# powdr-labs/powdr

Measured on AMD Instinct MI355X. Metric: STARK cells/sec (trace rows x cols) proving guest-keccak [bus interactions (LogUp) inside the proof], higher is better.
Workload: dtype u32 (BabyBear, Montgomery)

## Files before the change

include/powdr_prover.h:

```cpp
#ifndef POWDR_PROVER_H
#define POWDR_PROVER_H

#include <stddef.h>
#include <stdint.h>

#ifdef __cplusplus
extern "C" {
#endif

typedef struct PwProver PwProver;

typedef struct {
    uint32_t num_queries;
    uint32_t pow_bits;
} PwStarkConfig;

PwProver* pw_prover_create(const PwStarkConfig* cfg, uint32_t width, const uint32_t* cons_bytecode,
                           size_t bytecode_len, const uint32_t* cons_spans, size_t n_constraints);
PwProver* pw_prover_create_logup(const PwStarkConfig* cfg, uint32_t width, const uint32_t* cons_bytecode,
                                 size_t bytecode_len, const uint32_t* cons_spans, size_t n_constraints,
                                 const uint32_t* interactions, size_t n_interactions, const uint32_t* inter_spans,
                                 size_t n_inter_spans, const uint32_t* inter_bytecode, size_t inter_bytecode_len);
int pw_prover_trace_root(PwProver* p, const uint32_t* d_trace, uint32_t log_height, uint32_t* root8);
int pw_prover_set_bus_seed(PwProver* p, const uint32_t* seed8);
// ... 221 lines not shown
                               uint32_t* total_chunks);
void pw_jit_cache_stats(uint64_t* units_compiled, uint64_t* units_from_disk);
int pw_jit_compile_check(uint32_t width, const uint32_t* cons_bytecode, size_t bytecode_len, const uint32_t* cons_spans, size_t n_constraints,
                         const uint32_t* interactions, size_t n_interactions, const uint32_t* inter_spans, size_t n_inter_spans,
                         const uint32_t* inter_bytecode, size_t inter_bytecode_len, size_t* n_kernels, size_t* code_bytes, size_t* n_chunks,
                         char* err, size_t err_cap);

uint32_t pw_prover_width(const PwProver* p);

size_t pw_prover_device_bytes(const PwProver* p);


int pw_lde_batch(const uint32_t* d_trace, uint32_t width, uint32_t log_height, uint32_t* d_coeffs, uint32_t* d_lde);

int pw_lde_fused(const uint32_t* d_trace, uint32_t width, uint32_t log_height, uint32_t* d_tmp, uint32_t* d_lde);

int pw_lde_subcoset(const uint32_t* d_coeffs, uint32_t width, uint32_t log_height, uint32_t log_blocks, uint32_t r, uint32_t* d_scale,
                    uint32_t* d_out);

int pw_merkle_commit(const uint32_t* d_matrix, size_t height, uint32_t width, uint32_t* d_digests);

void pw_poseidon2_permute_host(uint32_t* state16);

int pw_set_poseidon2_constants(const uint32_t* ext_rc, const uint32_t* int_rc);
void pw_get_poseidon2_constants(uint32_t* ext_rc, uint32_t* int_rc, uint32_t* diag);

#ifdef __cplusplus
}
#endif
#endif
```

powdr_amd/csrc/field_selftest.hpp:

```cpp
#pragma once
#include "ext.hpp"
#include "poseidon2.hpp"

namespace pw {

PW_HD int field_selftest_checks(uint64_t seed, uint32_t iterations) {
    using namespace bb;
    uint64_t s = seed ? seed : 1;
    auto rnd = [&]() { s += 0x9E3779B97F4A7C15ull; uint64_t z = s; z = (z ^ (z >> 30)) * 0xBF58476D1CE4E5B9ull; z = (z ^ (z >> 27)) * 0x94D049BB133111EBull; return z ^ (z >> 31); };
    auto rp = [&]() { return (uint32_t)(rnd() % P); };
    const uint64_t edges64[] = {0, 1, P - 1, P, P + 1, 2ull * P - 1, 2ull * P, 16ull * P - 1, 75ull * P, 128ull * P - 1};
    for (uint64_t x : edges64) {
        if (x < 16ull * P && reduce_sum(x) != x % P) return 1;
        const uint32_t l = reduce_wide_loose(x);
        if (l % P != x % P || l >= (uint64_t)P + P / 32) return 2;
        if (reduce_wide(x) != x % P) return 3;
    }
    const uint32_t edges[] = {0, 1, P - 1, P, P + 1, 2 * P - 1};
    for (uint32_t a : edges)
        for (uint32_t b : edges) {
            const uint32_t r = add_2p(a, b), d = sub_2p(a, b);
            if (r >= 2 * P || r % P != (uint32_t)(((uint64_t)a + b) % P)) return 4;
            if (d >= 2 * P || d % P != (uint32_t)(((uint64_t)a + 2ull * P - b) % P)) return 5;
        }
// ... 26 lines not shown
        }
        const int32_t kappa = it < 3 ? ((it & 1) ? (int32_t)(P / 2) : -(int32_t)(P / 2)) : centred(rp());
        const int32_t rho = it < 3 ? ((it & 2) ? (int32_t)(P / 2) : -(int32_t)(P / 2)) : centred(rp());
        const uint32_t next = it < 3 ? P - 1 : rp(), ex = it < 3 ? (P + 1) / 2 : rp();
        int64_t exit_c[16];
        for (int i = 0; i < 16; ++i) exit_c[i] = (int64_t)centred(ex) * (int64_t)R_MOD_P;
        const bool last = it & 1;
        uint32_t wide = mul(mul(smodp(st[0]), smodp(kappa)), R2_MOD_P);
        for (int i = 1; i < 16; ++i) wide = add(wide, smodp(st[i]));
        const uint32_t sum = mul(wide, 1u);
        const uint32_t sum_r = mul(mul(sum, smodp(rho)), R2_MOD_P);
        for (int i = 0; i < 16; ++i) {
            const uint32_t prod = mul(mul(smodp(st[i]), smodp(m[i])), R2_MOD_P);
            const uint32_t c = i ? (last ? mul(mul(smodp(centred(ex)), R_MOD_P), R2_MOD_P) : 0u) : mul(mul(smodp(centred(next)), R_MOD_P), R2_MOD_P);
            want[i] = mul(add(add(sum_r, prod), c), 1u);
        }
        if (last) p2::internal_layer<true>(st, m, kappa, rho, (int64_t)centred(next) * (int64_t)R_MOD_P, exit_c);
        else p2::internal_layer<false>(st, m, kappa, rho, (int64_t)centred(next) * (int64_t)R_MOD_P, exit_c);
        for (int i = 0; i < 16; ++i)
            if (smodp(st[i]) != want[i]) return 9;
        for (int i = 0; i < 16; ++i)
            if (st[i] <= -(int32_t)P || st[i] >= (int32_t)P) return 9;
    }
    for (uint32_t it = 0; it < iterations; ++it) {
        const uint32_t a = rp(), b = rp(), c = rp(), d = rp();
        {
            const int32_t x = (int32_t)((int64_t)(rnd() % (2ull * P + P / 11)) - (int64_t)(P + P / 22));
            uint32_t want = R_MOD_P;
            for (int k = 0; k < 7; ++k) want = mul(want, smodp(x));
            if (smodp(p2::sbox7(x)) != want) return 8;
            const int64_t y = (int64_t)(rnd() % (128ull * P)) - 64ll * P;
            if (smodp(sreduce_wide_loose(y)) != smodp(y)) return 8;
        }
        const uint32_t ab = mul(a, b);
        if (ab >= P || (uint64_t)ab * R_MOD_P % P != (uint64_t)a * b % P) return 10;
        const uint32_t m2 = mul2(a, b, c, d);
        if (m2 != add(ab, mul(c, d))) return 11;
        const uint32_t la = (uint32_t)(rnd() % (2ull * P));
        const uint32_t ml = mul_lazy(la, b);
        if (ml >= 2 * P || ml % P != mul(la % P, b)) return 12;
        if (add_2p(la, (uint32_t)(rnd() % (2ull * P))) >= 2 * P) return 13;
        const uint64_t w = rnd() % (128ull * P);
        if (reduce_wide(w) != w % P) return 14;
        const uint32_t loose = reduce_wide_loose(w);
        if (loose % P != w % P || loose >= (uint64_t)P + P / 32) return 15;
        const uint64_t w16 = rnd() % (16ull * P);
// ... 49 lines not shown
```

powdr_amd/csrc/merkle.hip:

```cpp
#include "prover_internal.hpp"

#include <algorithm>
#include <cstdlib>
#include <mutex>

namespace pw {

namespace {

constexpr int kBlock = 256;
__constant__ p2::Params c_params;
p2::Params g_host_params;
bool g_params_ready = false;
uint64_t g_params_uploaded = 0;

template <int MINW>
__global__ __launch_bounds__(kBlock, MINW) void leaf_hash_kernel(const uint32_t* __restrict__ m, size_t height,
                                                            uint32_t width, size_t col_stride,
                                                            uint32_t* __restrict__ digests, size_t dstride, size_t doff) {
    const size_t j = (size_t)blockIdx.x * kBlock + threadIdx.x;
    if (j >= height) return;
    uint32_t st[16];
#pragma unroll
    for (int i = 0; i < 16; ++i) st[i] = 0u;
    const uint32_t* col = m + j;
#pragma unroll 1
    for (uint32_t c0 = 0; c0 < width; c0 += 8) {
#pragma unroll
        for (int k = 0; k < 8; ++k)
            if (c0 + k < width) st[k] = col[(size_t)(c0 + k) * col_stride];
        p2::permute<true>(st, c_params);
    }
#pragma unroll
    for (int k = 0; k < 8; ++k) st[k] = bb::reduce_2p(st[k]);
    uint4* out = reinterpret_cast<uint4*>(digests + (j * dstride + doff) * 8);
    out[0] = make_uint4(st[0], st[1], st[2], st[3]);
    out[1] = make_uint4(st[4], st[5], st[6], st[7]);
}

struct LeafLevel {
    const uint32_t* const* cols;
    uint32_t n_cols;
    uint32_t first_block;
    uint64_t height;
    uint32_t* out;
};
struct LeafLevels {
    LeafLevel lv[28];
    int n;
};
template <int MINW>
__global__ __launch_bounds__(kBlock, MINW) void leaf_hash_levels_kernel(const LeafLevels levels) {
    int k = 0;
    while (k + 1 < levels.n && blockIdx.x >= levels.lv[k + 1].first_block) ++k;
    const LeafLevel lv = levels.lv[k];
    const size_t j = (size_t)(blockIdx.x - lv.first_block) * kBlock + threadIdx.x;
    if (j >= lv.height) return;
    uint32_t st[16];
#pragma unroll
    for (int i = 0; i < 16; ++i) st[i] = 0u;
#pragma unroll 1
    for (uint32_t c0 = 0; c0 < lv.n_cols; c0 += 8) {
#pragma unroll
        for (int q = 0; q < 8; ++q)
            if (c0 + q < lv.n_cols) st[q] = lv.cols[c0 + q][j];
        p2::permute<true>(st, c_params);
    }
#pragma unroll
    for (int q = 0; q < 8; ++q) st[q] = bb::reduce_2p(st[q]);
    uint4* out = reinterpret_cast<uint4*>(lv.out + j * 8);
    out[0] = make_uint4(st[0], st[1], st[2], st[3]);
    out[1] = make_uint4(st[4], st[5], st[6], st[7]);
}

struct AbsorbArgs {
    const uint32_t* m;
    size_t col_stride;
    const uint32_t* const* cols;
    uint32_t n_cols, pos0;
    size_t height;
    size_t rstride, roff;
    uint32_t* state;
    uint32_t* digests;
    int first, last;
};
template <int MINW>
__global__ __launch_bounds__(kBlock, MINW) void leaf_absorb_kernel(const AbsorbArgs a) {
    const size_t j = (size_t)blockIdx.x * kBlock + threadIdx.x;
    if (j >= a.height) return;
    const size_t row = j * a.rstride + a.roff;
    uint32_t st[16];
    if (a.first) {
#pragma unroll
        for (int i = 0; i < 16; ++i) st[i] = 0u;
    } else {
        const uint4* in = reinterpret_cast<const uint4*>(a.state + row * 16);
#pragma unroll
        for (int v = 0; v < 4; ++v) { const uint4 x = in[v]; st[4 * v] = x.x; st[4 * v + 1] = x.y; st[4 * v + 2] = x.z; st[4 * v + 3] = x.w; }
    }
    auto cell = [&](uint32_t c) -> uint32_t { return a.cols ? a.cols[c][j] : a.m[(size_t)c * a.col_stride + j]; };
    uint32_t c = 0, pos = a.pos0;
    if (pos) {
#pragma unroll
        for (int k = 0; k < 8; ++k)
            if ((uint32_t)k >= pos && (uint32_t)k - pos < a.n_cols) st[k] = cell((uint32_t)k - pos);
        const uint32_t take = 8u - pos < a.n_cols ? 8u - pos : a.n_cols;
        c = take;
        pos += take;
        if (pos == 8u) { p2::permute<true>(st, c_params); pos = 0; }
    }
#pragma unroll 1
    for (; c < a.n_cols; c += 8) {
#pragma unroll
        for (int k = 0; k < 8; ++k)
            if (c + k < a.n_cols) st[k] = cell(c + k);
        if (c + 8 <= a.n_cols) p2::permute<true>(st, c_params);
        else pos = a.n_cols - c;
    }
    if (a.last) {
        if (pos) p2::permute<true>(st, c_params);
        uint4* out = reinterpret_cast<uint4*>(a.digests + row * 8);
        out[0] = make_uint4(bb::reduce_2p(st[0]), bb::reduce_2p(st[1]), bb::reduce_2p(st[2]), bb::reduce_2p(st[3]));
        out[1] = make_uint4(bb::reduce_2p(st[4]), bb::reduce_2p(st[5]), bb::reduce_2p(st[6]), bb::reduce_2p(st[7]));
    } else {
        uint4* out = reinterpret_cast<uint4*>(a.state + row * 16);
#pragma unroll
        for (int v = 0; v < 4; ++v) out[v] = make_uint4(st[4 * v], st[4 * v + 1], st[4 * v + 2], st[4 * v + 3]);
    }
}

__global__ __launch_bounds__(kBlock) void compress_strided_kernel(const uint32_t* __restrict__ children, size_t n,
                                                                   const uint32_t* __restrict__ inject, uint32_t* __restrict__ parents) {
    const size_t j = (size_t)blockIdx.x * kBlock + threadIdx.x;
    if (j >= n) return;
    const uint4* l = reinterpret_cast<const uint4*>(children + j * 8);
    const uint4* r = reinterpret_cast<const uint4*>(children + (j + n) * 8);
    uint4 a = l[0], b = l[1], c = r[0], d = r[1];
    uint32_t st[16] = {a.x, a.y, a.z, a.w, b.x, b.y, b.z, b.w, c.x, c.y, c.z, c.w, d.x, d.y, d.z, d.w};
    p2::permute(st, c_params);
    if (inject) {
        const uint4* q = reinterpret_cast<const uint4*>(inject + j * 8);
        c = q[0]; d = q[1];
        st[8] = c.x; st[9] = c.y; st[10] = c.z; st[11] = c.w; st[12] = d.x; st[13] = d.y; st[14] = d.z; st[15] = d.w;
        p2::permute(st, c_params);
    }
    uint4* out = reinterpret_cast<uint4*>(parents + j * 8);
    out[0] = make_uint4(st[0], st[1], st[2], st[3]);
    out[1] = make_uint4(st[4], st[5], st[6], st[7]);
}

__global__ __launch_bounds__(kBlock) void ext_pair_leaf_kernel(const bb::Ext* __restrict__ v, size_t half,
                                                                uint32_t* __restrict__ digests) {
    const size_t i = (size_t)blockIdx.x * kBlock + threadIdx.x;
    if (i >= half) return;
    uint32_t st[16];
    const bb::Ext a = v[i], b = v[i + half];
#pragma unroll
    for (int k = 0; k < 4; ++k) { st[k] = a.c[k]; st[4 + k] = b.c[k]; st[8 + k] = 0u; st[12 + k] = 0u; }
    p2::permute(st, c_params);
    uint4* out = reinterpret_cast<uint4*>(digests + i * 8);
    out[0] = make_uint4(st[0], st[1], st[2], st[3]);
    out[1] = make_uint4(st[4], st[5], st[6], st[7]);
}

__global__ __launch_bounds__(kBlock) void compress_kernel(const uint32_t* __restrict__ children, size_t n_parents,
                                                           uint32_t* __restrict__ parents) {
    const size_t i = (size_t)blockIdx.x * kBlock + threadIdx.x;
    if (i >= n_parents) return;
    const uint4* in = reinterpret_cast<const uint4*>(children + i * 16);
    uint4 a = in[0], b = in[1], c = in[2], d = in[3];
    uint32_t st[16] = {a.x, a.y, a.z, a.w, b.x, b.y, b.z, b.w, c.x, c.y, c.z, c.w, d.x, d.y, d.z, d.w};
    p2::permute(st, c_params);
    uint4* out = reinterpret_cast<uint4*>(parents + i * 8);
    out[0] = make_uint4(st[0], st[1], st[2], st[3]);
    out[1] = make_uint4(st[4], st[5], st[6], st[7]);
}

__global__ __launch_bounds__(kBlock) void pow_kernel(const uint32_t* __restrict__ state16, const uint32_t* __restrict__ pending,
                                                      uint32_t in_len, uint32_t bits, uint32_t base, uint32_t* best) {
    const uint32_t w = base + blockIdx.x * kBlock + threadIdx.x;
    if (w >= bb::P) return;
    uint32_t st[16];
#pragma unroll
    for (int i = 0; i < 16; ++i) st[i] = state16[i];
#pragma unroll
    for (int i = 0; i < 8; ++i)
        if ((uint32_t)i < in_len) st[i] = pending[i];
#pragma unroll
    for (int i = 0; i < 8; ++i)
        if ((uint32_t)i == in_len) st[i] = bb::to_monty(w);
    p2::permute(st, c_params);
    const uint32_t sample = st[7];
    if ((bb::from_monty(sample) & ((1u << bits) - 1u)) == 0u) atomicMin(best, w);
}

constexpr size_t kTailNodes = 2048;
__global__ __launch_bounds__(1024) void compress_tail_kernel(uint32_t* __restrict__ digests, size_t n_first, uint32_t* __restrict__ root_out) {
    size_t off = 0;
    for (size_t n = n_first; n > 1; n >>= 1) {
        const size_t parents = n >> 1;
        for (size_t i = threadIdx.x; i < parents; i += 1024) {
            const uint32_t* in = digests + off + i * 16;
            uint32_t st[16];
#pragma unroll
            for (int k = 0; k < 16; ++k) st[k] = in[k];
            p2::permute(st, c_params);
            uint32_t* out = digests + off + n * 8 + i * 8;
#pragma unroll
            for (int k = 0; k < 8; ++k) out[k] = st[k];
        }
        off += n * 8;
        __threadfence_block();
        __syncthreads();
    }
// ... 192 lines not shown
```

powdr_amd/csrc/poseidon2.hpp:

```cpp
#pragma once
#include "babybear.hpp"

#ifndef PW_P2_UNROLL
#define PW_P2_UNROLL 1
#endif
#define PW_P2_STR2(x) #x
#define PW_P2_STR(x) PW_P2_STR2(x)
#define PW_P2_ROUND_LOOP _Pragma(PW_P2_STR(unroll PW_P2_UNROLL))
#ifndef PW_P2_UNROLL_PARTIAL
#define PW_P2_UNROLL_PARTIAL 1
#endif
#define PW_P2_PARTIAL_LOOP _Pragma(PW_P2_STR(unroll PW_P2_UNROLL_PARTIAL))

namespace p2 {

struct Params {
    uint32_t ext_rc[8][16];
    uint32_t int_rc[13];
    uint32_t diag[16];
    int64_t ext_fold[8][16];
    int32_t entry_c;
    int32_t part_kappa[2];
    int32_t part_rho[2];
    int32_t part_diag[2][16];
// ... 73 lines not shown
        p.part_rho[k] = bb::centred((uint32_t)mulm(ratio, mulm(Rm, Rm)));
        for (int i = 0; i < 16; ++i) p.part_diag[k][i] = bb::centred((uint32_t)mulm(p.diag[i], i ? ratio : ratio0));
    }
    for (int r = 0; r < 13; ++r) {
        const uint32_t c = r < 12 ? p.int_rc[r + 1] : p.ext_rc[4][0];
        p.int_fold[r] = (int64_t)bb::centred((uint32_t)mulm(c, lam_second)) * (int64_t)bb::R_MOD_P;
    }
    for (int i = 0; i < 16; ++i) p.exit_fold[i] = i ? (int64_t)bb::centred((uint32_t)mulm(p.ext_rc[4][i], lam_second)) * (int64_t)bb::R_MOD_P : 0;
}

inline void generate_params(Params& p) {
    default_round_constants(p);
    derive_params(p);
}

PW_HD int32_t sbox7(int32_t x) {
    const int32_t x2 = bb::smont(bb::smul(x, x));
    const int32_t x3 = bb::smont(bb::smul(x2, x));
    const int32_t x4 = bb::smont(bb::smul(x2, x2));
    return bb::smont(bb::smul(x3, x4));
}

template <bool FOLD, bool BIAS>
PW_HD void external_layer(int32_t* s, const int64_t* fold) {
    int64_t y[16];
    constexpr int64_t kBias = 4 * (int64_t)bb::P;
#pragma unroll
    for (int b = 0; b < 4; ++b) {
        const int32_t x0 = s[4 * b], x1 = s[4 * b + 1], x2 = s[4 * b + 2], x3 = s[4 * b + 3];
        const int64_t t01 = bb::swide_add(FOLD ? bb::swide_fma_uniform(fold[4 * b], x0, 1) : BIAS ? bb::swide_fma_uniform(kBias, x0, 1) : bb::swide_mul(x0, 1), x1);
        const int64_t t23 = bb::swide_add(FOLD ? bb::swide_fma_uniform(fold[4 * b + 1], x2, 1) : BIAS ? bb::swide_fma_uniform(kBias, x2, 1) : bb::swide_mul(x2, 1), x3);
        const int64_t t = t01 + t23;
        const int64_t ta = bb::swide_add(t, x1), tb = bb::swide_add(t, x3);
        y[4 * b] = ta + t01;
        y[4 * b + 1] = bb::swide_fma(ta, x2, 2) + (FOLD ? fold[4 * b + 2] : (int64_t)0);
        y[4 * b + 2] = tb + t23;
        y[4 * b + 3] = bb::swide_fma(tb, x0, 2) + (FOLD ? fold[4 * b + 3] : (int64_t)0);
    }
#pragma unroll
    for (int i = 0; i < 4; ++i) {
        const int64_t col = (y[i] + y[4 + i]) + (y[8 + i] + y[12 + i]);
#pragma unroll
        for (int b = 0; b < 4; ++b) s[4 * b + i] = BIAS ? bb::sreduce_wide_loose(y[4 * b + i] + col) : bb::smont(y[4 * b + i] + col);
    }
}

template <bool LAST>
PW_HD void internal_layer(int32_t* s, const int32_t* m, int32_t kappa, int32_t rho, int64_t next_c, const int64_t* exit_c) {
    int64_t wide = bb::smul_uniform(s[0], kappa);
#pragma unroll
    for (int i = 1; i < 16; ++i) wide = bb::swide_add(wide, s[i]);
    const int32_t sum = bb::smont(wide);
    const int64_t sum_r = bb::smul_uniform(sum, rho);
    s[0] = bb::smont(bb::swide_mad_uniform(sum_r + next_c, s[0], m[0]));
#pragma unroll
    for (int i = 1; i < 16; ++i) s[i] = bb::smont(bb::swide_mad_uniform(LAST ? sum_r + exit_c[i] : sum_r, s[i], m[i]));
}

template <bool SPONGE = false>
PW_HD void permute(uint32_t* words, const Params& P) {
    int32_t* s = reinterpret_cast<int32_t*>(words);
    external_layer<true, false>(s, P.ext_fold[0]);
PW_P2_ROUND_LOOP
    for (int r = 0; r < 3; ++r) {
#pragma unroll
        for (int i = 0; i < 16; ++i) s[i] = sbox7(s[i]);
        external_layer<true, false>(s, P.ext_fold[r + 1]);
    }
#pragma unroll
    for (int i = 0; i < 16; ++i) s[i] = sbox7(s[i]);
    external_layer<false, false>(s, nullptr);
    s[0] += P.entry_c;
    s[0] = sbox7(s[0]);
    internal_layer<false>(s, P.part_diag[0], P.part_kappa[0], P.part_rho[0], P.int_fold[0], nullptr);
PW_P2_PARTIAL_LOOP
    for (int r = 1; r < 12; ++r) {
        s[0] = sbox7(s[0]);
        internal_layer<false>(s, P.part_diag[1], P.part_kappa[1], P.part_rho[1], P.int_fold[r], nullptr);
    }
    s[0] = sbox7(s[0]);
    internal_layer<true>(s, P.part_diag[1], P.part_kappa[1], P.part_rho[1], P.int_fold[12], P.exit_fold);
PW_P2_ROUND_LOOP
    for (int r = 4; r < 7; ++r) {
#pragma unroll
        for (int i = 0; i < 16; ++i) s[i] = sbox7(s[i]);
        external_layer<true, false>(s, P.ext_fold[r + 1]);
    }
#pragma unroll
    for (int i = 0; i < 16; ++i) s[i] = sbox7(s[i]);
    external_layer<false, true>(s, nullptr);
    if (!SPONGE) {
#pragma unroll
        for (int i = 0; i < 16; ++i) words[i] = bb::reduce_2p(words[i]);
    }
}

}
```

powdr_amd/csrc/prover.hip:

```cpp
#include "prover_state.hpp"
#include "prover_stages.hpp"
#include "xbc_compile.hpp"

#include <atomic>
#include <cstdlib>
#include <cstring>
#include <algorithm>
#include <initializer_list>
#include <vector>

namespace pw {

namespace {

__global__ void gather_records_kernel(const uint32_t* __restrict__ arena, const uint64_t* __restrict__ offsets,
                                      uint32_t words_per_record, uint32_t n, uint32_t* __restrict__ out) {
    const uint32_t i = blockIdx.x * blockDim.x + threadIdx.x;
    if (i >= n * words_per_record) return;
    const uint32_t r = i / words_per_record, w = i - r * words_per_record;
    out[i] = arena[offsets[r] + w];
}

}

// ... 942 lines not shown
extern "C" int pw_merkle_commit(const uint32_t* d_matrix, size_t height, uint32_t width, uint32_t* d_digests) {
    (void)hipGetLastError();
    if (!height || (height & (height - 1))) return -1;
    return merkle_commit_matrix(d_matrix, height, width, height, d_digests);
}

extern "C" int pw_set_poseidon2_constants(const uint32_t* ext_rc, const uint32_t* int_rc) {
    return poseidon2_set_constants(ext_rc, int_rc);
}

extern "C" void pw_get_poseidon2_constants(uint32_t* ext_rc, uint32_t* int_rc, uint32_t* diag) {
    const p2::Params& p = poseidon2_params_host();
    if (ext_rc) for (int r = 0; r < 8; ++r) for (int i = 0; i < 16; ++i) ext_rc[16 * r + i] = bb::from_monty(p.ext_rc[r][i]);
    if (int_rc) for (int r = 0; r < 13; ++r) int_rc[r] = bb::from_monty(p.int_rc[r]);
    if (diag) for (int i = 0; i < 16; ++i) diag[i] = bb::from_monty(p.diag[i]);
}

extern "C" void pw_poseidon2_permute_host(uint32_t* s) {
    uint32_t m[16];
    for (int i = 0; i < 16; ++i) m[i] = bb::to_monty(s[i] % bb::P);
    p2::permute(m, poseidon2_params_host());
    for (int i = 0; i < 16; ++i) s[i] = bb::from_monty(m[i]);
}
```

powdr_amd/prover.py:

```python
from __future__ import annotations

import ctypes as C

import numpy as np

from . import abi

lib = abi.lib


class PwStarkConfig(C.Structure):
    _fields_ = [("num_queries", C.c_uint32), ("pow_bits", C.c_uint32)]


PROVER_SYMBOLS = ["pw_prover_check_constraints", "pw_verify", "pw_prover_create", "pw_prover_create_logup", "pw_verify_logup", "pw_prover_trace_root", "pw_prover_set_bus_seed", "pw_prover_logup_path", "pw_prove_airs", "pw_verify_airs", "pw_prove_segment", "pw_verify_segment", "pw_commitment_digest", "pw_logup_group_starts", "pw_prover_width", "pw_prover_reserve", "pw_prover_stream_log_blocks", "pw_prover_max_constraint_degree", "pw_prover_destroy", "pw_prover_prove", "pw_prover_prove_consuming", "pw_prover_stream_log_blocks_consuming", "pw_trace_from_coefficients", "pw_prover_device_bytes",
                  "pw_lde_batch", "pw_lde_fused", "pw_lde_subcoset", "pw_merkle_commit", "pw_poseidon2_permute_host",
                  "pw_set_poseidon2_constants", "pw_get_poseidon2_constants", "pw_prover_specialise", "pw_prover_specialised", "pw_jit_compile_check", "pw_jit_cache_stats", "pw_jit_generated_source",
                  "pw_prove_segments_multi", "pw_multi_last_merge", "pw_assign_units",
                  "pw_prove_segment_consuming", "pw_segment_last_modes", "pw_segment_last_plan", "pw_set_device_budget", "pw_get_device_budget", "pw_provers_specialise",
                  "pw_segment_context_bytes", "pw_segment_stream_plan", "pw_segment_last_plan_tables",
                  "pw_prover_create_preprocessed", "pw_prover_preprocessed_root", "pw_prover_preprocessed_width", "pw_verify_segment_preprocessed",
                  "pw_prover_create_transition", "pw_prover_row_flags", "pw_verify_segment_transition",
                  "pw_prover_create_public", "pw_prover_n_public", "pw_prover_set_public_values", "pw_verify_segment_public",
                  "pw_segment_proof_public_values", "pw_verify_segment_chain", "pw_public_programs_check",
                  "pw_check_segment_buses", "pw_bus_check_scratch_bytes", "pw_bus_check_peak_bytes", "pw_bus_check_last_stats",
                  "pw_poseidon2_compress_trace",
                  "pw_memory_tree_create", "pw_memory_tree_destroy", "pw_memory_tree_root", "pw_memory_tree_stats", "pw_memory_tree_update",
                  "pw_memory_tree_boundary_leaves", "pw_memory_tree_set_mode", "pw_memory_tree_get_mode",
                  "pw_memory_merkle_trace", "pw_memory_tree_open", "pw_memory_opening_verify"]

lib.pw_prover_create.restype = C.c_void_p
lib.pw_prover_create.argtypes = [C.POINTER(PwStarkConfig), C.c_uint32, C.c_void_p, C.c_size_t, C.c_void_p, C.c_size_t]
lib.pw_prover_create_logup.restype = C.c_void_p
lib.pw_prover_create_logup.argtypes = [C.POINTER(PwStarkConfig), C.c_uint32, C.c_void_p, C.c_size_t, C.c_void_p, C.c_size_t,
                                       C.c_void_p, C.c_size_t, C.c_void_p, C.c_size_t, C.c_void_p, C.c_size_t]
lib.pw_prover_destroy.argtypes = [C.c_void_p]
lib.pw_prover_create_preprocessed.restype = C.c_void_p
lib.pw_prover_create_preprocessed.argtypes = [C.POINTER(PwStarkConfig), C.c_uint32, C.c_uint32, C.c_uint32, C.c_void_p, C.c_void_p, C.c_size_t,
                                              C.c_void_p, C.c_size_t, C.c_void_p, C.c_size_t, C.c_void_p, C.c_size_t, C.c_void_p, C.c_size_t]
# ... 24 lines not shown
lib.pw_lde_fused.argtypes = [C.c_void_p, C.c_uint32, C.c_uint32, C.c_void_p, C.c_void_p]
lib.pw_prover_prove_consuming.restype = C.c_int
lib.pw_prover_prove_consuming.argtypes = lib.pw_prover_prove.argtypes
lib.pw_prover_stream_log_blocks_consuming.restype = C.c_int
lib.pw_prover_stream_log_blocks_consuming.argtypes = [C.c_void_p, C.c_uint32]
lib.pw_trace_from_coefficients.restype = C.c_int
lib.pw_trace_from_coefficients.argtypes = [C.c_void_p, C.c_uint32, C.c_uint32, C.c_void_p]
lib.pw_lde_subcoset.restype = C.c_int
lib.pw_lde_subcoset.argtypes = [C.c_void_p, C.c_uint32, C.c_uint32, C.c_uint32, C.c_uint32, C.c_void_p, C.c_void_p]
lib.pw_segment_last_modes.restype = C.c_size_t
lib.pw_segment_last_modes.argtypes = [C.c_void_p, C.c_size_t]
lib.pw_segment_context_bytes.restype = C.c_size_t
lib.pw_segment_context_bytes.argtypes = []
lib.pw_segment_stream_plan.restype = C.c_size_t
lib.pw_segment_stream_plan.argtypes = [C.c_size_t, C.c_void_p, C.c_void_p, C.c_void_p, C.c_size_t, C.c_size_t, C.c_void_p]
lib.pw_segment_last_plan_tables.restype = C.c_size_t
lib.pw_segment_last_plan_tables.argtypes = [C.c_void_p, C.c_void_p, C.c_void_p, C.c_size_t]
lib.pw_set_device_budget.restype = None
lib.pw_set_device_budget.argtypes = [C.c_size_t]
lib.pw_get_device_budget.restype = C.c_size_t
lib.pw_merkle_commit.restype = C.c_int
lib.pw_merkle_commit.argtypes = [C.c_void_p, C.c_size_t, C.c_uint32, C.c_void_p]
lib.pw_poseidon2_permute_host.argtypes = [C.c_void_p]


def _vp(a):
    return a.ctypes.data_as(C.c_void_p)


def _interaction_tables(interactions):
    if interactions is None:
        return (None, 0, None, 0, None, 0), []
    it = np.ascontiguousarray(interactions[0], dtype=np.uint32).reshape(-1, 3)
    isp = np.ascontiguousarray(interactions[1], dtype=np.uint32).reshape(-1, 2)
    ibc = np.ascontiguousarray(interactions[2], dtype=np.uint32)
    return (_vp(it), len(it), _vp(isp), len(isp), _vp(ibc), len(ibc)), [it, isp, ibc]


lib.pw_verify.restype = C.c_int
lib.pw_verify.argtypes = [C.POINTER(PwStarkConfig), C.c_uint32, C.c_uint32, C.c_void_p, C.c_size_t, C.c_void_p, C.c_size_t,
                          C.c_void_p, C.c_size_t]


def verify(proof, width: int, log_height: int, cons_bytecode, cons_spans, num_queries: int = 100, pow_bits: int = 0) -> int:
    pr = np.ascontiguousarray(proof, dtype=np.uint32)
    bc = np.ascontiguousarray(cons_bytecode, dtype=np.uint32)
# ... 400 lines not shown
    xbc, src = np.zeros(max(nx.value, 1), np.uint32), C.create_string_buffer(ns.value + 1)
    lib.pw_public_programs_check(*args, _vp(xbc), nx.value, C.byref(nx), src, ns.value + 1, C.byref(ns))
    return dict(max_degree=deg.value, row_flags=rf.value, xbc=xbc[:nx.value].copy(), source=src.value.decode())


def verify_airs(descs, proofs, num_queries: int = 100, pow_bits: int = 0, shared_bus_seed: bool = False, check_balance: bool = False):
    n = len(descs)
    recs, keep = _air_descriptions(descs)
    prs = [np.ascontiguousarray(p, dtype=np.uint32) for p in proofs]
    ptrs = (C.c_void_p * max(n, 1))(*[p.ctypes.data for p in prs])
    lens = (C.c_size_t * max(n, 1))(*[len(p) for p in prs])
    cfg = PwStarkConfig(num_queries, pow_bits)
    total = np.zeros(4, np.uint32)
    rc = int(lib.pw_verify_airs(C.byref(cfg), recs, n, ptrs, lens, int(shared_bus_seed), int(check_balance), _vp(total)))
    return rc, total


def poseidon2_host(state) -> np.ndarray:
    s = np.ascontiguousarray(state, dtype=np.uint32).copy()
    lib.pw_poseidon2_permute_host(s.ctypes.data_as(C.c_void_p))
    return s


lib.pw_set_poseidon2_constants.restype = C.c_int
lib.pw_set_poseidon2_constants.argtypes = [C.c_void_p, C.c_void_p]
lib.pw_get_poseidon2_constants.restype = None
lib.pw_get_poseidon2_constants.argtypes = [C.c_void_p, C.c_void_p, C.c_void_p]


def jit_compile_check(width: int, cons_bytecode, cons_spans, interactions=None) -> dict:
    vp = lambda a: a.ctypes.data_as(C.c_void_p)
    bc = np.ascontiguousarray(cons_bytecode, dtype=np.uint32)
    sp = np.ascontiguousarray(cons_spans, dtype=np.uint32).reshape(-1, 2)
    k, b, c = C.c_size_t(), C.c_size_t(), C.c_size_t()
    err = C.create_string_buffer(4096)
    f = lib.pw_jit_compile_check
    f.restype = C.c_int
    f.argtypes = [C.c_uint32, C.c_void_p, C.c_size_t, C.c_void_p, C.c_size_t, C.c_void_p, C.c_size_t, C.c_void_p, C.c_size_t, C.c_void_p, C.c_size_t,
                  C.POINTER(C.c_size_t), C.POINTER(C.c_size_t), C.POINTER(C.c_size_t), C.c_char_p, C.c_size_t]
    tables, _ = _interaction_tables(interactions)
    rc = f(width, vp(bc), len(bc), vp(sp), len(sp), *tables, C.byref(k), C.byref(b), C.byref(c), err, 4096)
    return dict(rc=int(rc), kernels=k.value, code_bytes=b.value, chunks=c.value, error=err.value.decode(errors="replace"))


def jit_generated_sources(width: int, cons_bytecode, cons_spans, interactions=None, which: int = 0, chunk_cost: int = 0, chunks_per_unit: int = 0):
    vp = lambda a: a.ctypes.data_as(C.c_void_p)
# ... 215 lines not shown
```

rust/powdr-hip/src/ffi.rs:

```rust
#![allow(non_camel_case_types, clippy::too_many_arguments)]

use core::ffi::{c_char, c_int, c_uint, c_void};

pub type PowdrFp = u32;

#[repr(C)]
#[derive(Clone, Copy, Debug)]
pub struct OriginalAir {
    pub width: i32,
    pub height: i32,
    pub buffer: *const PowdrFp,
    pub row_block_size: i32,
}
#[repr(C)]
#[derive(Clone, Copy, Debug)]
pub struct Subst {
    pub air_index: i32,
    pub col: i32,
    pub row: i32,
    pub apc_col: i32,
}
#[repr(C)]
#[derive(Clone, Copy)]
pub struct ExprSpan {
// ... 436 lines not shown
    pub fn pw_prover_width(p: *const PwProver) -> u32;
    pub fn pw_prover_device_bytes(p: *const PwProver) -> usize;
    pub fn pw_lde_batch(d_trace: *const u32, width: u32, log_height: u32, d_coeffs: *mut u32, d_lde: *mut u32) -> c_int;
    pub fn pw_lde_fused(d_trace: *const u32, width: u32, log_height: u32, d_tmp: *mut u32, d_lde: *mut u32) -> c_int;
    pub fn pw_lde_subcoset(d_coeffs: *const u32, width: u32, log_height: u32, log_blocks: u32, r: u32, d_scale: *mut u32, d_out: *mut u32) -> c_int;
    pub fn pw_merkle_commit(d_matrix: *const u32, height: usize, width: u32, d_digests: *mut u32) -> c_int;
    pub fn pw_prover_specialise(p: *mut PwProver) -> c_int;
    pub fn pw_prover_specialised(p: *const PwProver, n_kernels: *mut usize, code_bytes: *mut usize, n_chunks: *mut usize) -> c_int;
    pub fn pw_prove_segments_multi(devices: *const c_int, n_workers: usize, segment_cells: *const u64, n_segments: usize,
                                   prove: PwSegmentProveFn, user: *mut c_void, commitments: *mut u32, worker_of_segment: *mut u32) -> c_int;
    pub fn pw_multi_last_merge() -> c_int;
    pub fn pw_assign_units(cells: *const u64, n_units: usize, n_workers: usize, worker_of_unit: *mut u32) -> usize;
    pub fn pw_jit_generated_source(width: u32, cons_bytecode: *const u32, bytecode_len: usize, cons_spans: *const u32, n_constraints: usize,
                                   interactions: *const u32, n_interactions: usize, inter_spans: *const u32, n_inter_spans: usize,
                                   inter_bytecode: *const u32, inter_bytecode_len: usize, which: c_int, chunk_cost: u32, chunks_per_unit: u32,
                                   unit: usize, buf: *mut c_char, cap: usize, kernel_name: *mut c_char, name_cap: usize, first_chunk: *mut u32,
                                   n_chunks: *mut u32, total_chunks: *mut u32) -> usize;
    pub fn pw_jit_cache_stats(units_compiled: *mut u64, units_from_disk: *mut u64);
    pub fn pw_jit_compile_check(width: u32, cons_bytecode: *const u32, bytecode_len: usize, cons_spans: *const u32, n_constraints: usize,
                                interactions: *const u32, n_interactions: usize, inter_spans: *const u32, n_inter_spans: usize,
                                inter_bytecode: *const u32, inter_bytecode_len: usize, n_kernels: *mut usize, code_bytes: *mut usize,
                                n_chunks: *mut usize, err: *mut c_char, err_cap: usize) -> c_int;
    pub fn pw_poseidon2_permute_host(state16: *mut u32);
    pub fn pw_set_poseidon2_constants(ext_rc: *const u32, int_rc: *const u32) -> c_int;
    pub fn pw_get_poseidon2_constants(ext_rc: *mut u32, int_rc: *mut u32, diag: *mut u32);
}

extern "C" {
    pub fn hipMalloc(ptr: *mut *mut c_void, bytes: usize) -> c_int;
    pub fn hipFree(ptr: *mut c_void) -> c_int;
    pub fn hipMemcpy(dst: *mut c_void, src: *const c_void, bytes: usize, kind: c_int) -> c_int;
    pub fn hipMemset(dst: *mut c_void, value: c_int, bytes: usize) -> c_int;
    pub fn hipDeviceSynchronize() -> c_int;
    pub fn hipSetDevice(device: c_int) -> c_int;
}
pub const HIP_MEMCPY_HOST_TO_DEVICE: c_int = 1;
pub const HIP_MEMCPY_DEVICE_TO_HOST: c_int = 2;
```

Baseline: 7.142 billion.

## Specialise Poseidon2 first/last layers for sponge absorption and 2-to-1 compression

```diff
diff --git a/include/powdr_prover.h b/include/powdr_prover.h
--- a/include/powdr_prover.h
+++ b/include/powdr_prover.h
@@ -267,6 +267,10 @@
 
 void pw_poseidon2_permute_host(uint32_t* state16);
 
+void pw_poseidon2_sponge_host(const uint32_t* words, uint32_t n_words, const uint32_t* runs, uint32_t n_runs, uint32_t* digest8);
+void pw_poseidon2_compress_host(const uint32_t* left_right16, uint32_t* node8);
+uint64_t pw_poseidon2_sponge_capacity_host(const uint32_t* words, uint32_t n_words);
+
 int pw_set_poseidon2_constants(const uint32_t* ext_rc, const uint32_t* int_rc);
 void pw_get_poseidon2_constants(uint32_t* ext_rc, uint32_t* int_rc, uint32_t* diag);
 
diff --git a/powdr_amd/csrc/field_selftest.hpp b/powdr_amd/csrc/field_selftest.hpp
--- a/powdr_amd/csrc/field_selftest.hpp
+++ b/powdr_amd/csrc/field_selftest.hpp
@@ -72,6 +72,40 @@
         for (int i = 0; i < 16; ++i)
             if (st[i] <= -(int32_t)P || st[i] >= (int32_t)P) return 9;
     }
+    for (uint32_t it = 0; it < 6 + iterations / 16; ++it) {
+        const int32_t top = (int32_t)((uint64_t)P * 93 / 100);
+        int32_t sx[16], full[16], dig[16];
+        for (int i = 0; i < 16; ++i) {
+            const int32_t mag = it < 4 ? top - 1 : (int32_t)(rnd() % (uint64_t)top);
+            sx[i] = it == 0 ? mag : it == 1 ? -mag : it == 2 ? ((i & 1) ? mag : -mag) : it == 3 ? ((i & 4) ? mag : -mag) : ((rnd() & 1) ? mag : -mag);
+            full[i] = dig[i] = sx[i];
+        }
+        p2::external_layer<false, true>(full, nullptr);
+        int64_t cap[8];
+        p2::last_layer_capacity(sx, cap);
+        p2::last_layer_digest(dig);
+        for (int k = 0; k < 8; ++k) {
+            if (smodp(cap[k]) != smodp(full[8 + k]) || cap[k] <= -33ll * P || cap[k] >= 33ll * P) return 26;
+            if (smodp(dig[k]) != smodp(full[k]) || dig[k] < 0 || dig[k] >= (int32_t)(P + P / 50)) return 27;
+        }
+        if (it == 0 && cap[0] < 32ll * P) return 26;
+        if (it == 1 && cap[0] > -32ll * P) return 26;
+        int32_t rate[8], ref[16], got[16];
+        int64_t wide[8], fold[16];
+        for (int k = 0; k < 8; ++k) {
+            const int64_t cmag = it < 4 ? 33ll * P - 1 : (int64_t)(rnd() % (33ull * P));
+            wide[k] = it == 4 || it == 5 ? (int64_t)(it == 4 ? 0 : P + P / 50) : it == 0 ? cmag : it == 1 ? -cmag : ((k + it) & 1) ? cmag : -cmag;
+            rate[k] = it == 0 || it == 5 ? (int32_t)(P + P / 50) : it == 1 ? 0 : it < 4 ? (int32_t)(P - 1) : (int32_t)rp();
+            ref[k] = rate[k];
+            ref[8 + k] = (int32_t)smodp(wide[k]);
+        }
+        auto uni = [](uint64_t k) { uint64_t z = (k + 1) * 0x9E3779B97F4A7C15ull; z = (z ^ (z >> 30)) * 0xBF58476D1CE4E5B9ull; z = (z ^ (z >> 27)) * 0x94D049BB133111EBull; return z ^ (z >> 31); };
+        for (int i = 0; i < 16; ++i) fold[i] = it < 4 ? ((i + it) & 1 ? (int64_t)(P / 2) : -(int64_t)(P / 2)) : (int64_t)centred((uint32_t)(uni(16ull * it + i) % P));
+        p2::external_layer<true, false>(ref, fold);
+        p2::first_layer_sponge(rate, wide, got, fold);
+        for (int i = 0; i < 16; ++i)
+            if (smodp(got[i]) != smodp(ref[i]) || got[i] <= -(int32_t)(P / 2 + 1024) || got[i] >= (int32_t)(P / 2 + 1024)) return 28;
+    }
     for (uint32_t it = 0; it < iterations; ++it) {
         const uint32_t a = rp(), b = rp(), c = rp(), d = rp();
         {
diff --git a/powdr_amd/csrc/merkle.hip b/powdr_amd/csrc/merkle.hip
--- a/powdr_amd/csrc/merkle.hip
+++ b/powdr_amd/csrc/merkle.hip
@@ -20,19 +20,9 @@
                                                             uint32_t* __restrict__ digests, size_t dstride, size_t doff) {
     const size_t j = (size_t)blockIdx.x * kBlock + threadIdx.x;
     if (j >= height) return;
-    uint32_t st[16];
-#pragma unroll
-    for (int i = 0; i < 16; ++i) st[i] = 0u;
     const uint32_t* col = m + j;
-#pragma unroll 1
-    for (uint32_t c0 = 0; c0 < width; c0 += 8) {
-#pragma unroll
-        for (int k = 0; k < 8; ++k)
-            if (c0 + k < width) st[k] = col[(size_t)(c0 + k) * col_stride];
-        p2::permute<true>(st, c_params);
-    }
-#pragma unroll
-    for (int k = 0; k < 8; ++k) st[k] = bb::reduce_2p(st[k]);
+    uint32_t st[8];
+    p2::sponge_hash_row(width, [&](uint32_t c) { return col[(size_t)c * col_stride]; }, c_params, st);
     uint4* out = reinterpret_cast<uint4*>(digests + (j * dstride + doff) * 8);
     out[0] = make_uint4(st[0], st[1], st[2], st[3]);
     out[1] = make_uint4(st[4], st[5], st[6], st[7]);
@@ -56,18 +46,8 @@
     const LeafLevel lv = levels.lv[k];
     const size_t j = (size_t)(blockIdx.x - lv.first_block) * kBlock + threadIdx.x;
     if (j >= lv.height) return;
-    uint32_t st[16];
-#pragma unroll
-    for (int i = 0; i < 16; ++i) st[i] = 0u;
-#pragma unroll 1
-    for (uint32_t c0 = 0; c0 < lv.n_cols; c0 += 8) {
-#pragma unroll
-        for (int q = 0; q < 8; ++q)
-            if (c0 + q < lv.n_cols) st[q] = lv.cols[c0 + q][j];
-        p2::permute<true>(st, c_params);
-    }
-#pragma unroll
-    for (int q = 0; q < 8; ++q) st[q] = bb::reduce_2p(st[q]);
+    uint32_t st[8];
+    p2::sponge_hash_row(lv.n_cols, [&](uint32_t c) { return lv.cols[c][j]; }, c_params, st);
     uint4* out = reinterpret_cast<uint4*>(lv.out + j * 8);
     out[0] = make_uint4(st[0], st[1], st[2], st[3]);
     out[1] = make_uint4(st[4], st[5], st[6], st[7]);
@@ -90,39 +70,24 @@
     if (j >= a.height) return;
     const size_t row = j * a.rstride + a.roff;
     uint32_t st[16];
+    p2::Sponge sp;
     if (a.first) {
-#pragma unroll
-        for (int i = 0; i < 16; ++i) st[i] = 0u;
+        p2::sponge_init(sp);
     } else {
         const uint4* in = reinterpret_cast<const uint4*>(a.state + row * 16);
 #pragma unroll
         for (int v = 0; v < 4; ++v) { const uint4 x = in[v]; st[4 * v] = x.x; st[4 * v + 1] = x.y; st[4 * v + 2] = x.z; st[4 * v + 3] = x.w; }
+        p2::sponge_load(sp, st);
     }
     auto cell = [&](uint32_t c) -> uint32_t { return a.cols ? a.cols[c][j] : a.m[(size_t)c * a.col_stride + j]; };
-    uint32_t c = 0, pos = a.pos0;
-    if (pos) {
-#pragma unroll
-        for (int k = 0; k < 8; ++k)
-            if ((uint32_t)k >= pos && (uint32_t)k - pos < a.n_cols) st[k] = cell((uint32_t)k - pos);
-        const uint32_t take = 8u - pos < a.n_cols ? 8u - pos : a.n_cols;
-        c = take;
-        pos += take;
-        if (pos == 8u) { p2::permute<true>(st, c_params); pos = 0; }
-    }
-#pragma unroll 1
-    for (; c < a.n_cols; c += 8) {
-#pragma unroll
-        for (int k = 0; k < 8; ++k)
-            if (c + k < a.n_cols) st[k] = cell(c + k);
-        if (c + 8 <= a.n_cols) p2::permute<true>(st, c_params);
-        else pos = a.n_cols - c;
-    }
+    const uint32_t pos = p2::sponge_absorb_run(sp, a.n_cols, a.pos0, cell, c_params);
     if (a.last) {
-        if (pos) p2::permute<true>(st, c_params);
+        p2::sponge_close(sp, pos, c_params, st);
         uint4* out = reinterpret_cast<uint4*>(a.digests + row * 8);
-        out[0] = make_uint4(bb::reduce_2p(st[0]), bb::reduce_2p(st[1]), bb::reduce_2p(st[2]), bb::reduce_2p(st[3]));
-        out[1] = make_uint4(bb::reduce_2p(st[4]), bb::reduce_2p(st[5]), bb::reduce_2p(st[6]), bb::reduce_2p(st[7]));
+        out[0] = make_uint4(st[0], st[1], st[2], st[3]);
+        out[1] = make_uint4(st[4], st[5], st[6], st[7]);
     } else {
+        p2::sponge_store(sp, st);
         uint4* out = reinterpret_cast<uint4*>(a.state + row * 16);
 #pragma unroll
         for (int v = 0; v < 4; ++v) out[v] = make_uint4(st[4 * v], st[4 * v + 1], st[4 * v + 2], st[4 * v + 3]);
@@ -137,12 +102,12 @@
     const uint4* r = reinterpret_cast<const uint4*>(children + (j + n) * 8);
     uint4 a = l[0], b = l[1], c = r[0], d = r[1];
     uint32_t st[16] = {a.x, a.y, a.z, a.w, b.x, b.y, b.z, b.w, c.x, c.y, c.z, c.w, d.x, d.y, d.z, d.w};
-    p2::permute(st, c_params);
+    p2::permute_compress(st, c_params);
     if (inject) {
         const uint4* q = reinterpret_cast<const uint4*>(inject + j * 8);
         c = q[0]; d = q[1];
         st[8] = c.x; st[9] = c.y; st[10] = c.z; st[11] = c.w; st[12] = d.x; st[13] = d.y; st[14] = d.z; st[15] = d.w;
-        p2::permute(st, c_params);
+        p2::permute_compress(st, c_params);
     }
     uint4* out = reinterpret_cast<uint4*>(parents + j * 8);
     out[0] = make_uint4(st[0], st[1], st[2], st[3]);
@@ -157,7 +122,7 @@
     const bb::Ext a = v[i], b = v[i + half];
 #pragma unroll
     for (int k = 0; k < 4; ++k) { st[k] = a.c[k]; st[4 + k] = b.c[k]; st[8 + k] = 0u; st[12 + k] = 0u; }
-    p2::permute(st, c_params);
+    p2::permute_compress(st, c_params);
     uint4* out = reinterpret_cast<uint4*>(digests + i * 8);
     out[0] = make_uint4(st[0], st[1], st[2], st[3]);
     out[1] = make_uint4(st[4], st[5], st[6], st[7]);
@@ -170,7 +135,7 @@
     const uint4* in = reinterpret_cast<const uint4*>(children + i * 16);
     uint4 a = in[0], b = in[1], c = in[2], d = in[3];
     uint32_t st[16] = {a.x, a.y, a.z, a.w, b.x, b.y, b.z, b.w, c.x, c.y, c.z, c.w, d.x, d.y, d.z, d.w};
-    p2::permute(st, c_params);
+    p2::permute_compress(st, c_params);
     uint4* out = reinterpret_cast<uint4*>(parents + i * 8);
     out[0] = make_uint4(st[0], st[1], st[2], st[3]);
     out[1] = make_uint4(st[4], st[5], st[6], st[7]);
@@ -189,7 +154,7 @@
 #pragma unroll
     for (int i = 0; i < 8; ++i)
         if ((uint32_t)i == in_len) st[i] = bb::to_monty(w);
-    p2::permute(st, c_params);
+    p2::permute_compress(st, c_params);
     const uint32_t sample = st[7];
     if ((bb::from_monty(sample) & ((1u << bits) - 1u)) == 0u) atomicMin(best, w);
 }
diff --git a/powdr_amd/csrc/poseidon2.hpp b/powdr_amd/csrc/poseidon2.hpp
--- a/powdr_amd/csrc/poseidon2.hpp
+++ b/powdr_amd/csrc/poseidon2.hpp
@@ -119,6 +119,31 @@
 }
 
 template <bool FOLD, bool BIAS>
+PW_HD void m4_block(const int32_t* x, const int64_t* fold, int64_t* y) {
+    constexpr int64_t kBias = 4 * (int64_t)bb::P;
+    const int32_t x0 = x[0], x1 = x[1], x2 = x[2], x3 = x[3];
+    const int64_t t01 = bb::swide_add(FOLD ? bb::swide_fma_uniform(fold[0], x0, 1) : BIAS ? bb::swide_fma_uniform(kBias, x0, 1) : bb::swide_mul(x0, 1), x1);
+    const int64_t t23 = bb::swide_add(FOLD ? bb::swide_fma_uniform(fold[1], x2, 1) : BIAS ? bb::swide_fma_uniform(kBias, x2, 1) : bb::swide_mul(x2, 1), x3);
+    const int64_t t = t01 + t23;
+    const int64_t ta = bb::swide_add(t, x1), tb = bb::swide_add(t, x3);
+    y[0] = ta + t01;
+    y[1] = bb::swide_fma(ta, x2, 2) + (FOLD ? fold[2] : (int64_t)0);
+    y[2] = tb + t23;
+    y[3] = bb::swide_fma(tb, x0, 2) + (FOLD ? fold[3] : (int64_t)0);
+}
+template <bool FOLD>
+PW_HD void m4_block_wide(const int64_t* z, const int64_t* fold, int64_t* y) {
+    const int64_t t01 = (FOLD ? z[0] + fold[0] : z[0]) + z[1];
+    const int64_t t23 = (FOLD ? z[2] + fold[1] : z[2]) + z[3];
+    const int64_t t = t01 + t23;
+    const int64_t ta = t + z[1], tb = t + z[3];
+    y[0] = ta + t01;
+    y[1] = (ta + 2 * z[2]) + (FOLD ? fold[2] : (int64_t)0);
+    y[2] = tb + t23;
+    y[3] = (tb + 2 * z[0]) + (FOLD ? fold[3] : (int64_t)0);
+}
+
+template <bool FOLD, bool BIAS>
 PW_HD void external_layer(int32_t* s, const int64_t* fold) {
     int64_t y[16];
     constexpr int64_t kBias = 4 * (int64_t)bb::P;
@@ -142,6 +167,47 @@
     }
 }
 
+PW_HD void last_layer_capacity(const int32_t* s, int64_t* cap) {
+    int64_t X[4];
+#pragma unroll
+    for (int i = 0; i < 4; ++i) X[i] = bb::swide_add(bb::swide_add(bb::swide_add(bb::swide_mul(s[i], 1), s[4 + i]), s[8 + i]), s[12 + i]);
+#pragma unroll
+    for (int b = 2; b < 4; ++b) {
+        int64_t z[4];
+#pragma unroll
+        for (int i = 0; i < 4; ++i) z[i] = bb::swide_add(X[i], s[4 * b + i]);
+        m4_block_wide<false>(z, nullptr, cap + 4 * (b - 2));
+    }
+}
+PW_HD void last_layer_digest(int32_t* s) {
+    constexpr int64_t kBias = 5 * (int64_t)bb::P;
+    int64_t X[4];
+#pragma unroll
+    for (int i = 0; i < 4; ++i) X[i] = bb::swide_add(bb::swide_add(bb::swide_add(bb::swide_fma_uniform(kBias, s[i], 1), s[4 + i]), s[8 + i]), s[12 + i]);
+#pragma unroll
+    for (int b = 0; b < 2; ++b) {
+        int64_t z[4], y[4];
+#pragma unroll
+        for (int i = 0; i < 4; ++i) z[i] = bb::swide_add(X[i], s[4 * b + i]);
+        m4_block_wide<false>(z, nullptr, y);
+#pragma unroll
+        for (int i = 0; i < 4; ++i) s[4 * b + i] = bb::sreduce_wide_loose(y[i]);
+    }
+}
+PW_HD void first_layer_sponge(const int32_t* rate, const int64_t* cap, int32_t* s, const int64_t* fold) {
+    int64_t y[16];
+#pragma unroll
+    for (int b = 0; b < 2; ++b) m4_block<true, false>(rate + 4 * b, fold + 4 * b, y + 4 * b);
+#pragma unroll
+    for (int b = 2; b < 4; ++b) m4_block_wide<true>(cap + 4 * (b - 2), fold + 4 * b, y + 4 * b);
+#pragma unroll
+    for (int i = 0; i < 4; ++i) {
+        const int64_t col = (y[i] + y[4 + i]) + (y[8 + i] + y[12 + i]);
+#pragma unroll
+        for (int b = 0; b < 4; ++b) s[4 * b + i] = bb::smont(y[4 * b + i] + col);
+    }
+}
+
 template <bool LAST>
 PW_HD void internal_layer(int32_t* s, const int32_t* m, int32_t kappa, int32_t rho, int64_t next_c, const int64_t* exit_c) {
     int64_t wide = bb::smul_uniform(s[0], kappa);
@@ -154,37 +220,40 @@
     for (int i = 1; i < 16; ++i) s[i] = bb::smont(bb::swide_mad_uniform(LAST ? sum_r + exit_c[i] : sum_r, s[i], m[i]));
 }
 
+#define PW_P2_ROUNDS(s, P) \
+PW_P2_ROUND_LOOP \
+    for (int r = 0; r < 3; ++r) { \
+_Pragma("unroll") \
+        for (int i = 0; i < 16; ++i) s[i] = sbox7(s[i]); \
+        external_layer<true, false>(s, P.ext_fold[r + 1]); \
+    } \
+_Pragma("unroll") \
+    for (int i = 0; i < 16; ++i) s[i] = sbox7(s[i]); \
+    external_layer<false, false>(s, nullptr); \
+    s[0] += P.entry_c; \
+    s[0] = sbox7(s[0]); \
+    internal_layer<false>(s, P.part_diag[0], P.part_kappa[0], P.part_rho[0], P.int_fold[0], nullptr); \
+PW_P2_PARTIAL_LOOP \
+    for (int r = 1; r < 12; ++r) { \
+        s[0] = sbox7(s[0]); \
+        internal_layer<false>(s, P.part_diag[1], P.part_kappa[1], P.part_rho[1], P.int_fold[r], nullptr); \
+    } \
+    s[0] = sbox7(s[0]); \
+    internal_layer<true>(s, P.part_diag[1], P.part_kappa[1], P.part_rho[1], P.int_fold[12], P.exit_fold); \
+PW_P2_ROUND_LOOP \
+    for (int r = 4; r < 7; ++r) { \
+_Pragma("unroll") \
+        for (int i = 0; i < 16; ++i) s[i] = sbox7(s[i]); \
+        external_layer<true, false>(s, P.ext_fold[r + 1]); \
+    } \
+_Pragma("unroll") \
+    for (int i = 0; i < 16; ++i) s[i] = sbox7(s[i]);
+
 template <bool SPONGE = false>
 PW_HD void permute(uint32_t* words, const Params& P) {
     int32_t* s = reinterpret_cast<int32_t*>(words);
     external_layer<true, false>(s, P.ext_fold[0]);
-PW_P2_ROUND_LOOP
-    for (int r = 0; r < 3; ++r) {
-#pragma unroll
-        for (int i = 0; i < 16; ++i) s[i] = sbox7(s[i]);
-        external_layer<true, false>(s, P.ext_fold[r + 1]);
-    }
-#pragma unroll
-    for (int i = 0; i < 16; ++i) s[i] = sbox7(s[i]);
-    external_layer<false, false>(s, nullptr);
-    s[0] += P.entry_c;
-    s[0] = sbox7(s[0]);
-    internal_layer<false>(s, P.part_diag[0], P.part_kappa[0], P.part_rho[0], P.int_fold[0], nullptr);
-PW_P2_PARTIAL_LOOP
-    for (int r = 1; r < 12; ++r) {
-        s[0] = sbox7(s[0]);
-        internal_layer<false>(s, P.part_diag[1], P.part_kappa[1], P.part_rho[1], P.int_fold[r], nullptr);
-    }
-    s[0] = sbox7(s[0]);
-    internal_layer<true>(s, P.part_diag[1], P.part_kappa[1], P.part_rho[1], P.int_fold[12], P.exit_fold);
-PW_P2_ROUND_LOOP
-    for (int r = 4; r < 7; ++r) {
-#pragma unroll
-        for (int i = 0; i < 16; ++i) s[i] = sbox7(s[i]);
-        external_layer<true, false>(s, P.ext_fold[r + 1]);
-    }
-#pragma unroll
-    for (int i = 0; i < 16; ++i) s[i] = sbox7(s[i]);
+    PW_P2_ROUNDS(s, P)
     external_layer<false, true>(s, nullptr);
     if (!SPONGE) {
 #pragma unroll
@@ -192,4 +261,88 @@
     }
 }
 
-}
+PW_HD void permute_compress(uint32_t* words, const Params& P) {
+    int32_t* s = reinterpret_cast<int32_t*>(words);
+    external_layer<true, false>(s, P.ext_fold[0]);
+    PW_P2_ROUNDS(s, P)
+    last_layer_digest(s);
+#pragma unroll
+    for (int i = 0; i < 8; ++i) words[i] = bb::reduce_2p(words[i]);
+}
+
+struct Sponge {
+    int32_t rate[8];
+    int64_t cap[8];
+};
+PW_HD void sponge_init(Sponge& sp) {
+#pragma unroll
+    for (int k = 0; k < 8; ++k) { sp.rate[k] = 0; sp.cap[k] = 0; }
+}
+PW_HD void sponge_permute(Sponge& sp, bool keep_rate, const Params& P) {
+    int32_t s[16];
+    first_layer_sponge(sp.rate, sp.cap, s, P.ext_fold[0]);
+    PW_P2_ROUNDS(s, P)
+    if (keep_rate) {
+        external_layer<false, true>(s, nullptr);
+#pragma unroll
+        for (int k = 0; k < 8; ++k) sp.cap[k] = s[8 + k];
+    } else {
+        last_layer_capacity(s, sp.cap);
+    }
+#pragma unroll
+    for (int k = 0; k < 8; ++k) sp.rate[k] = s[k];
+}
+PW_HD void sponge_load(Sponge& sp, const uint32_t* st16) {
+#pragma unroll
+    for (int k = 0; k < 8; ++k) { sp.rate[k] = (int32_t)st16[k]; sp.cap[k] = (int32_t)st16[8 + k]; }
+}
+PW_HD void sponge_store(const Sponge& sp, uint32_t* st16) {
+#pragma unroll
+    for (int k = 0; k < 8; ++k) { st16[k] = (uint32_t)sp.rate[k]; st16[8 + k] = (uint32_t)sp.cap[k]; }
+}
+PW_HD void sponge_digest(const Sponge& sp, uint32_t* digest8) {
+#pragma unroll
+    for (int k = 0; k < 8; ++k) digest8[k] = bb::reduce_2p((uint32_t)sp.rate[k]);
+}
+
+template <class Cell>
+PW_HD void sponge_hash_row(uint32_t width, Cell&& cell, const Params& P, uint32_t* digest8) {
+    Sponge sp;
+    sponge_init(sp);
+#pragma unroll 1
+    for (uint32_t c0 = 0; c0 < width; c0 += 8) {
+#pragma unroll
+        for (int k = 0; k < 8; ++k)
+            if (c0 + k < width) sp.rate[k] = (int32_t)cell(c0 + k);
+        sponge_permute(sp, width - c0 < 16u, P);
+    }
+    sponge_digest(sp, digest8);
+}
+template <class Cell>
+PW_HD uint32_t sponge_absorb_run(Sponge& sp, uint32_t n_cols, uint32_t pos0, Cell&& cell, const Params& P) {
+    uint32_t c = 0, pos = pos0;
+    if (pos) {
+#pragma unroll
+        for (int k = 0; k < 8; ++k)
+            if ((uint32_t)k >= pos && (uint32_t)k - pos < n_cols) sp.rate[k] = (int32_t)cell((uint32_t)k - pos);
+        const uint32_t take = 8u - pos < n_cols ? 8u - pos : n_cols;
+        c = take;
+        pos += take;
+        if (pos == 8u) { sponge_permute(sp, n_cols - c < 8u, P); pos = 0; }
+    }
+#pragma unroll 1
+    for (; c < n_cols; c += 8) {
+#pragma unroll
+        for (int k = 0; k < 8; ++k)
+            if (c + k < n_cols) sp.rate[k] = (int32_t)cell(c + k);
+        if (c + 8 <= n_cols) sponge_permute(sp, n_cols - c < 16u, P);
+        else pos = n_cols - c;
+    }
+    return pos;
+}
+PW_HD void sponge_close(Sponge& sp, uint32_t pos, const Params& P, uint32_t* digest8) {
+    if (pos) sponge_permute(sp, true, P);
+    sponge_digest(sp, digest8);
+}
+
+}
diff --git a/powdr_amd/csrc/prover.hip b/powdr_amd/csrc/prover.hip
--- a/powdr_amd/csrc/prover.hip
+++ b/powdr_amd/csrc/prover.hip
@@ -988,3 +988,45 @@
     p2::permute(m, poseidon2_params_host());
     for (int i = 0; i < 16; ++i) s[i] = bb::from_monty(m[i]);
 }
+
+extern "C" void pw_poseidon2_sponge_host(const uint32_t* words, uint32_t n_words, const uint32_t* runs, uint32_t n_runs, uint32_t* digest8) {
+    const p2::Params& P = poseidon2_params_host();
+    uint32_t d[8];
+    if (!n_runs) {
+        p2::sponge_hash_row(n_words, [&](uint32_t c) { return bb::to_monty(words[c] % bb::P); }, P, d);
+    } else {
+        uint32_t parked[16] = {0}, pos = 0, off = 0;
+        for (uint32_t r = 0; r < n_runs; ++r) {
+            p2::Sponge sp;
+            p2::sponge_load(sp, parked);
+            const uint32_t len = runs[r] < n_words - off ? runs[r] : n_words - off;
+            pos = p2::sponge_absorb_run(sp, len, pos, [&](uint32_t c) { return bb::to_monty(words[off + c] % bb::P); }, P);
+            off += len;
+            if (r + 1 == n_runs) p2::sponge_close(sp, pos, P, d);
+            else p2::sponge_store(sp, parked);
+        }
+    }
+    for (int i = 0; i < 8; ++i) digest8[i] = bb::from_monty(d[i]);
+}
+
+extern "C" uint64_t pw_poseidon2_sponge_capacity_host(const uint32_t* words, uint32_t n_words) {
+    const p2::Params& P = poseidon2_params_host();
+    p2::Sponge sp;
+    p2::sponge_init(sp);
+    uint64_t worst = 0;
+    for (uint32_t c0 = 0; c0 < n_words; c0 += 8) {
+        for (uint32_t k = 0; k < 8 && c0 + k < n_words; ++k) sp.rate[k] = (int32_t)bb::to_monty(words[c0 + k] % bb::P);
+        const bool keep_rate = n_words - c0 < 16u;
+        p2::sponge_permute(sp, keep_rate, P);
+        if (!keep_rate)
+            for (int k = 0; k < 8; ++k) { const uint64_t m = (uint64_t)(sp.cap[k] < 0 ? -sp.cap[k] : sp.cap[k]); if (m > worst) worst = m; }
+    }
+    return worst;
+}
+
+extern "C" void pw_poseidon2_compress_host(const uint32_t* left_right16, uint32_t* node8) {
+    uint32_t m[16];
+    for (int i = 0; i < 16; ++i) m[i] = bb::to_monty(left_right16[i] % bb::P);
+    p2::permute_compress(m, poseidon2_params_host());
+    for (int i = 0; i < 8; ++i) node8[i] = bb::from_monty(m[i]);
+}
diff --git a/powdr_amd/prover.py b/powdr_amd/prover.py
--- a/powdr_amd/prover.py
+++ b/powdr_amd/prover.py
@@ -14,7 +14,7 @@
 
 
 PROVER_SYMBOLS = ["pw_prover_check_constraints", "pw_verify", "pw_prover_create", "pw_prover_create_logup", "pw_verify_logup", "pw_prover_trace_root", "pw_prover_set_bus_seed", "pw_prover_logup_path", "pw_prove_airs", "pw_verify_airs", "pw_prove_segment", "pw_verify_segment", "pw_commitment_digest", "pw_logup_group_starts", "pw_prover_width", "pw_prover_reserve", "pw_prover_stream_log_blocks", "pw_prover_max_constraint_degree", "pw_prover_destroy", "pw_prover_prove", "pw_prover_prove_consuming", "pw_prover_stream_log_blocks_consuming", "pw_trace_from_coefficients", "pw_prover_device_bytes",
-                  "pw_lde_batch", "pw_lde_fused", "pw_lde_subcoset", "pw_merkle_commit", "pw_poseidon2_permute_host",
+                  "pw_lde_batch", "pw_lde_fused", "pw_lde_subcoset", "pw_merkle_commit", "pw_poseidon2_permute_host", "pw_poseidon2_sponge_host", "pw_poseidon2_compress_host", "pw_poseidon2_sponge_capacity_host",
                   "pw_set_poseidon2_constants", "pw_get_poseidon2_constants", "pw_prover_specialise", "pw_prover_specialised", "pw_jit_compile_check", "pw_jit_cache_stats", "pw_jit_generated_source",
                   "pw_prove_segments_multi", "pw_multi_last_merge", "pw_assign_units",
                   "pw_prove_segment_consuming", "pw_segment_last_modes", "pw_segment_last_plan", "pw_set_device_budget", "pw_get_device_budget", "pw_provers_specialise",
@@ -85,6 +85,12 @@
 lib.pw_merkle_commit.restype = C.c_int
 lib.pw_merkle_commit.argtypes = [C.c_void_p, C.c_size_t, C.c_uint32, C.c_void_p]
 lib.pw_poseidon2_permute_host.argtypes = [C.c_void_p]
+lib.pw_poseidon2_sponge_host.restype = None
+lib.pw_poseidon2_sponge_host.argtypes = [C.c_void_p, C.c_uint32, C.c_void_p, C.c_uint32, C.c_void_p]
+lib.pw_poseidon2_sponge_capacity_host.restype = C.c_uint64
+lib.pw_poseidon2_sponge_capacity_host.argtypes = [C.c_void_p, C.c_uint32]
+lib.pw_poseidon2_compress_host.restype = None
+lib.pw_poseidon2_compress_host.argtypes = [C.c_void_p, C.c_void_p]
 
 
 def _vp(a):
@@ -531,6 +537,27 @@
     return s
 
 
+def poseidon2_sponge_host(words, runs=None) -> np.ndarray:
+    w = np.ascontiguousarray(words, dtype=np.uint32)
+    r = np.ascontiguousarray(runs if runs is not None else [], dtype=np.uint32)
+    out = np.zeros(8, np.uint32)
+    lib.pw_poseidon2_sponge_host(_vp(w), len(w), _vp(r), len(r), _vp(out))
+    return out
+
+
+def poseidon2_sponge_capacity_host(words) -> int:
+    w = np.ascontiguousarray(words, dtype=np.uint32)
+    return int(lib.pw_poseidon2_sponge_capacity_host(_vp(w), len(w)))
+
+
+def poseidon2_compress_host(left_right16) -> np.ndarray:
+    s = np.ascontiguousarray(left_right16, dtype=np.uint32)
+    assert len(s) == 16
+    out = np.zeros(8, np.uint32)
+    lib.pw_poseidon2_compress_host(_vp(s), _vp(out))
+    return out
+
+
 lib.pw_set_poseidon2_constants.restype = C.c_int
 lib.pw_set_poseidon2_constants.argtypes = [C.c_void_p, C.c_void_p]
 lib.pw_get_poseidon2_constants.restype = None
diff --git a/rust/powdr-hip/src/ffi.rs b/rust/powdr-hip/src/ffi.rs
--- a/rust/powdr-hip/src/ffi.rs
+++ b/rust/powdr-hip/src/ffi.rs
@@ -482,6 +482,9 @@
                                 inter_bytecode: *const u32, inter_bytecode_len: usize, n_kernels: *mut usize, code_bytes: *mut usize,
                                 n_chunks: *mut usize, err: *mut c_char, err_cap: usize) -> c_int;
     pub fn pw_poseidon2_permute_host(state16: *mut u32);
+    pub fn pw_poseidon2_sponge_host(words: *const u32, n_words: u32, runs: *const u32, n_runs: u32, digest8: *mut u32);
+    pub fn pw_poseidon2_compress_host(left_right16: *const u32, node8: *mut u32);
+    pub fn pw_poseidon2_sponge_capacity_host(words: *const u32, n_words: u32) -> u64;
     pub fn pw_set_poseidon2_constants(ext_rc: *const u32, int_rc: *const u32) -> c_int;
     pub fn pw_get_poseidon2_constants(ext_rc: *mut u32, int_rc: *mut u32, diag: *mut u32);
 }
```

Result: no change. 7.212 billion (median of 6 runs) (+1.0%).
